# florasion/D-VQVAE

Measured on NVIDIA B200. Metric: vq_latents_per_sec, higher is better.
Workload: dtype f32

## Files before the change

### d-vqvae_b200/csrc/dvq_api.cu

```cuda
#include <dlfcn.h>
#include <stdarg.h>
#include <stdlib.h>
#include <string.h>

#include "dvq_common.cuh"

namespace dvq {

static thread_local char g_err[512] = "";

void set_error(const char* fmt, ...) {
  va_list ap;
  va_start(ap, fmt);
  vsnprintf(g_err, sizeof(g_err), fmt, ap);
  va_end(ap);
}

int fail(int code, const char* fmt, ...) {
  va_list ap;
  va_start(ap, fmt);
  vsnprintf(g_err, sizeof(g_err), fmt, ap);
  va_end(ap);
  return code;
}

int device_props(DeviceProps* out) {
  static DeviceProps cache[64];
  static bool have[64] = {};
  int dev = 0;
  DVQ_CUDA_CHECK(cudaGetDevice(&dev));
  if (dev < 0 || dev >= 64) return fail(DVQ_ERR_CUDA, "device ordinal %d out of range", dev);
  if (!have[dev]) {
    DeviceProps p;
    DVQ_CUDA_CHECK(cudaDeviceGetAttribute(&p.sm_count, cudaDevAttrMultiProcessorCount, dev));
    DVQ_CUDA_CHECK(cudaDeviceGetAttribute(&p.cc_major, cudaDevAttrComputeCapabilityMajor, dev));
    DVQ_CUDA_CHECK(cudaDeviceGetAttribute(&p.cc_minor, cudaDevAttrComputeCapabilityMinor, dev));
    DVQ_CUDA_CHECK(cudaDeviceGetAttribute(&p.max_smem_optin, cudaDevAttrMaxSharedMemoryPerBlockOptin, dev));
    cache[dev] = p;
    have[dev] = true;
  }
  *out = cache[dev];
  return DVQ_OK;
}

static long long g_launches = 0;
void count_launch(int n) { __atomic_fetch_add(&g_launches, (long long)n, __ATOMIC_RELAXED); }

static int g_refine_mode = 0;
static long long g_refine_pair_cap = 0;
long long refine_pair_cap_override() { return __atomic_load_n(&g_refine_pair_cap, __ATOMIC_RELAXED); }

static const int kStages = 4;
static const int kProfSlots = 128;
static thread_local bool g_prof_on = false;
static thread_local cudaEvent_t g_prof_ev[kStages][kProfSlots][2] = {};
static thread_local int g_prof_n[kStages] = {};

void profile_mark(int stage, bool begin, cudaStream_t s) {
  if (!g_prof_on || stage < 0 || stage >= kStages) return;
  const int slot = g_prof_n[stage];
  if (slot >= kProfSlots) return;
  cudaEvent_t& e = g_prof_ev[stage][slot][begin ? 0 : 1];
  if (!e && cudaEventCreate(&e) != cudaSuccess) return;
  cudaEventRecord(e, s);
  if (!begin) g_prof_n[stage] = slot + 1;
}

static int require_sm100() {
  DeviceProps dp;
  int rc = device_props(&dp);
  if (rc) return rc;
  if (dp.cc_major != 10)
    return fail(DVQ_ERR_UNSUPPORTED_ARCH, "libdvq_sm100 is built for sm_100a only; device is sm_%d%d",
                dp.cc_major, dp.cc_minor);
  return DVQ_OK;
}

VqWorkspace vq_workspace_layout(int64_t N, int K, int D, int flags) {
  VqWorkspace w;
  size_t off = 0;
  w.off_ee = off;
  off = align_up(off + sizeof(float) * (size_t)K, 256);
  w.off_counters = off;
  off = align_up(off + sizeof(int) * 64, 256);
  const bool may_tc = (flags & DVQ_PATH_MASK) != DVQ_PATH_SIMT && vq_tc_supported(N, K, D);
  w.off_rowlist = off;
  if (may_tc) off = align_up(off + 2 * align_up(sizeof(int) * (size_t)N, 256), 256);
  w.off_bop = off;
  if (may_tc) off = align_up(off + vq_tc_operand_bytes(K, D), 1024);
  w.off_binned = off;
  if (may_tc) off = align_up(off + vq_refine_binned_bytes(N), 256);
  w.total = off;
  return w;
}

}

using namespace dvq;

extern "C" {

int dvq_abi_version(void) { return DVQ_ABI_VERSION; }

const char* dvq_last_error(void) { return g_err; }

long long dvq_launch_count(void) { return __atomic_load_n(&g_launches, __ATOMIC_RELAXED); }

int dvq_vq_set_refine(int mode, long long pair_cap) {
  if (mode < 0 || mode > 2) return fail(DVQ_ERR_BAD_ARG, "refine mode must be 0 (auto), 1 (per-row) or 2 (binned)");
  __atomic_store_n(&g_refine_mode, mode, __ATOMIC_RELAXED);
  __atomic_store_n(&g_refine_pair_cap, pair_cap > 0 ? pair_cap : 0, __ATOMIC_RELAXED);
  return DVQ_OK;
}

int dvq_debug_tc_layout(int K, int D, int* out8) {
  if (!out8) return fail(DVQ_ERR_BAD_ARG, "out8 is NULL");
  if (K <= 0 || D <= 0) return fail(DVQ_ERR_BAD_SHAPE, "need K > 0, D > 0");
  vq_tc_layout_info(K, D, out8);
  return DVQ_OK;
}

int dvq_debug_tc_pair_layout(long long N, int K, int D, int* out8) {
  if (!out8) return fail(DVQ_ERR_BAD_ARG, "out8 is NULL");
  if (K <= 0 || D <= 0) return fail(DVQ_ERR_BAD_SHAPE, "need K > 0, D > 0");
  vq_tc_pair_layout_info((int64_t)N, K, D, out8);
  return DVQ_OK;
}

int dvq_debug_tc_layout_ex(long long N, int K, int D, int flags, int* out8) {
  if (!out8) return fail(DVQ_ERR_BAD_ARG, "out8 is NULL");
  if (K <= 0 || D <= 0) return fail(DVQ_ERR_BAD_SHAPE, "need K > 0, D > 0");
  const int zbytes = (flags & DVQ_Z_BF16) ? 2 : 4;
  if (vq_tc_pair_selected((int64_t)N, K, D)) vq_tc_pair_layout_info((int64_t)N, K, D, out8, zbytes);
  else vq_tc_layout_info(K, D, out8, zbytes);
  return DVQ_OK;
}

long long dvq_debug_tc_image_offset(int k, int d, int K, int D, int pair, long long* image_bytes) {
  if (K <= 0 || D <= 0 || k < 0 || k >= K || d < 0 || d >= D + 16 || !vq_tc_supported(1, K, D)) return -1;
  return vq_tc_image_offset(k, d, K, D, pair, image_bytes);
}

int dvq_profile_enable(int on) {
  g_prof_on = on != 0;
  for (int i = 0; i < kStages; ++i) g_prof_n[i] = 0;
  return DVQ_OK;
}

int dvq_profile_mean(float* ms, int* count, int n) {
  if (!ms || n <= 0) return fail(DVQ_ERR_BAD_ARG, "ms is NULL or n <= 0");
  for (int i = 0; i < n; ++i) {
    ms[i] = 0.f;
    if (count) count[i] = 0;
    if (i >= kStages) continue;
    double sum = 0.0;
    for (int j = 0; j < g_prof_n[i]; ++j) {
      float t = 0.f;
      DVQ_CUDA_CHECK(cudaEventSynchronize(g_prof_ev[i][j][1]));
      DVQ_CUDA_CHECK(cudaEventElapsedTime(&t, g_prof_ev[i][j][0], g_prof_ev[i][j][1]));
      sum += t;
    }
    if (g_prof_n[i] > 0) ms[i] = (float)(sum / g_prof_n[i]);
    if (count) count[i] = g_prof_n[i];
  }
  return DVQ_OK;
}

int dvq_device_info(int* sm_count, int* cc_major, int* cc_minor) {
  DeviceProps dp;
  int rc = device_props(&dp);
  if (rc) return rc;
  if (sm_count) *sm_count = dp.sm_count;
  if (cc_major) *cc_major = dp.cc_major;
  if (cc_minor) *cc_minor = dp.cc_minor;
  return DVQ_OK;
}

static int check_vq_shape(int64_t N, int K, int D) {
  if (N < 0 || K <= 0 || D <= 0) return fail(DVQ_ERR_BAD_SHAPE, "need N >= 0, K > 0, D > 0 (got N=%lld K=%d D=%d)", (long long)N, K, D);
  if (N > 2147483647LL - 256) return fail(DVQ_ERR_BAD_SHAPE, "N=%lld exceeds the per-call limit of 2^31-257 rows; shard the call", (long long)N);
  return DVQ_OK;
}

int dvq_vq_workspace_bytes(int64_t N, int K, int D, int flags, size_t* bytes) {
  if (!bytes) return fail(DVQ_ERR_BAD_ARG, "bytes is NULL");
  int rc = check_vq_shape(N, K, D);
  if (rc) return rc;
  *bytes = vq_workspace_layout(N, K, D, flags).total;
  return DVQ_OK;
}

int dvq_vq_forward(const float* z, const float* E, int64_t N, int K, int D, int flags, float* z_q, int64_t* idx,
                   float* onehot, unsigned long long* hist, double* sse, void* workspace, size_t workspace_bytes,
                   void* stream) {
  int rc = check_vq_shape(N, K, D);
  if (rc) return rc;
  const int train = (flags & DVQ_TRAIN) ? 1 : 0;
  if (!E || !workspace) return fail(DVQ_ERR_BAD_ARG, "E / workspace must not be NULL");
  if (N > 0 && (!z || !z_q || !idx)) return fail(DVQ_ERR_BAD_ARG, "z, z_q and idx must not be NULL");
  if (train && (!hist || !sse)) return fail(DVQ_ERR_BAD_ARG, "DVQ_TRAIN needs hist and sse");
  if ((flags & DVQ_WRITE_ONEHOT) && !onehot) return fail(DVQ_ERR_BAD_ARG, "DVQ_WRITE_ONEHOT needs onehot");
  const bool zbf = (flags & DVQ_Z_BF16) != 0;
  if ((reinterpret_cast<uintptr_t>(z) | reinterpret_cast<uintptr_t>(z_q)) % (zbf ? 2 : 4) != 0 || reinterpret_cast<uintptr_t>(E) % 4 != 0 ||
      reinterpret_cast<uintptr_t>(idx) % 8 != 0 || reinterpret_cast<uintptr_t>(workspace) % 256 != 0)
    return fail(DVQ_ERR_BAD_ALIGN, "z/z_q need %d-byte, E 4-byte, idx 8-byte, workspace 256-byte alignment", zbf ? 2 : 4);
  const VqWorkspace w = vq_workspace_layout(N, K, D, flags);
  if (workspace_bytes < w.total)
    return fail(DVQ_ERR_WORKSPACE, "workspace too small: %zu < %zu bytes", workspace_bytes, w.total);
  rc = require_sm100();
  if (rc) return rc;
  cudaStream_t s = static_cast<cudaStream_t>(stream);
  char* ws = static_cast<char*>(workspace);
  float* ee = reinterpret_cast<float*>(ws + w.off_ee);

  const int path = flags & DVQ_PATH_MASK;
  const bool tc_ok = vq_tc_supported(N, K, D);
  if (path == DVQ_PATH_TC && !tc_ok)
    return fail(DVQ_ERR_BAD_SHAPE, "DVQ_PATH_TC: shape N=%lld K=%d D=%d is not handled by the tcgen05 kernel", (long long)N, K, D);
  const bool aligned16 = (reinterpret_cast<uintptr_t>(z) | reinterpret_cast<uintptr_t>(E) | reinterpret_cast<uintptr_t>(z_q)) % 16 == 0;
  const bool use_tc = tc_ok && path != DVQ_PATH_SIMT && (aligned16 || path == DVQ_PATH_TC);

  const bool cached = (flags & DVQ_CODEBOOK_CACHED) != 0;
  profile_mark(0, true, s);
  if (!cached) rc = launch_code_norms(E, K, D, ee, s);
  profile_mark(0, false, s);
  if (rc) return rc;
  if (N > 0) {
    if (use_tc) {
      int* counters = reinterpret_cast<int*>(ws + w.off_counters);
      int* row_list = reinterpret_cast<int*>(ws + w.off_rowlist);
      int* cand_list = reinterpret_cast<int*>(ws + w.off_rowlist + align_up(sizeof(int) * (size_t)N, 256));
      profile_mark(1, true, s);
      rc = launch_vq_tc(z, E, ee, N, K, D, train, z_q, idx, hist, sse, ws + w.off_bop, counters, row_list, cand_list,
                        reinterpret_cast<int*>(ws + w.off_binned), (int)(vq_refine_binned_zero_bytes() / sizeof(int)), cached, zbf, s);
      profile_mark(1, false, s);
      if (rc) return rc;
      profile_mark(2, true, s);
      const bool list_mode = vq_tc_cand_gshift(K) < 0;
      if (vq_refine_supported(K, D)) {
        static const bool env_per_row = getenv("DVQ_REFINE_PER_ROW") != nullptr;
        static const bool env_binned = getenv("DVQ_REFINE_BINNED") != nullptr;
        const int mode = __atomic_load_n(&g_refine_mode, __ATOMIC_RELAXED);
        const bool force_per_row = env_per_row || mode == 1, force_binned = env_binned || mode == 2;
        const bool per_row_only = force_per_row || (!force_binned && vq_refine_codebook_in_smem(K, D));
        if (!per_row_only)
          rc = launch_vq_refine_binned(z, E, ee, N, K, D, train, z_q, idx, hist, sse, row_list, cand_list, counters, list_mode ? 1 : 0,
                                       ws + w.off_binned, zbf, s);
        if (!rc)
          rc = launch_vq_refine(z, E, ee, K, D, train, z_q, idx, hist, sse, row_list, cand_list, per_row_only ? counters : counters + 5,
                                vq_tc_cand_gshift(K), list_mode ? row_list + (N - 1) : nullptr,
                                list_mode ? (per_row_only ? counters + 2 : counters + 6) : nullptr, zbf, s);
      } else {
        rc = launch_vq_simt(z, E, ee, N, K, D, train, z_q, idx, hist, sse, row_list, counters, 1, zbf, s);
        if (!rc && list_mode)
          rc = launch_vq_simt(z, E, ee, N, K, D, train, z_q, idx, hist, sse, row_list + (N - 1), counters + 2, -1, zbf, s);
      }
      profile_mark(2, false, s);
      if (rc) return rc;
    } else {
      profile_mark(1, true, s);
      rc = launch_vq_simt(z, E, ee, N, K, D, train, z_q, idx, hist, sse, nullptr, nullptr, 1, zbf, s);
      profile_mark(1, false, s);
      if (rc) return rc;
    }
    if (flags & DVQ_WRITE_ONEHOT) {
      profile_mark(3, true, s);
      rc = launch_onehot(idx, N, K, onehot, s);
      profile_mark(3, false, s);
      if (rc) return rc;
    }
  }
  return DVQ_OK;
}

int dvq_vq_read_counters(const void* workspace, int64_t N, int K, int D, int flags, int* out4) {
  if (!workspace || !out4) return fail(DVQ_ERR_BAD_ARG, "NULL argument");
  int rc = check_vq_shape(N, K, D);
  if (rc) return rc;
  out4[0] = out4[1] = out4[2] = out4[3] = 0;
  const bool use_tc = vq_tc_supported(N, K, D) && (flags & DVQ_PATH_MASK) != DVQ_PATH_SIMT;
  if (!use_tc) return DVQ_OK;
  const VqWorkspace w = vq_workspace_layout(N, K, D, flags);
  DVQ_CUDA_CHECK(cudaMemcpy(out4, static_cast<const char*>(workspace) + w.off_counters, 4 * sizeof(int), cudaMemcpyDeviceToHost));
  if (getenv("DVQ_TC_STATS_PRINT")) {
    unsigned long long st[17];
    DVQ_CUDA_CHECK(cudaMemcpy(st, static_cast<const char*>(workspace) + w.off_counters + 32, sizeof(st), cudaMemcpyDeviceToHost));
    static const char* names[17] = {"producer.wait_stage_empty", "mma.wait_a_full", "mma.wait_acc_empty", "mma.total",
                                    "conv.wait_stage_full", "conv.wait_a_empty", "conv.total", "epi0.wait_acc_full",
                                    "epi4.wait_fin_empty", "epi0.wait_fin_full", "epi0.wait_sidx_empty", "epi0.total",
                                    "gather.wait_sidx_full", "gather.total", "mma.wait_b_full", "(unused)", "mma.wait_peer_acc_empty"};
    for (int i = 0; i < 17; ++i) fprintf(stderr, "[dvq tc stats] %-28s %14llu cycles (sum over CTAs)\n", names[i], st[i]);
    if (N >= 65536) {
      static long long tr[5 * 8 * 8];
      DVQ_CUDA_CHECK(cudaMemcpy(tr, static_cast<const char*>(workspace) + w.off_rowlist + (size_t)(N - 8192) * sizeof(int), sizeof(tr),
                                cudaMemcpyDeviceToHost));
      static const char* ev[5][4] = {{"mma.a_full", "mma.acc_empty", "mma.issued", "mma.complete"},
                                     {"own.acc_full", "own.chunk_done", "own.fin_full", "own.sidx_out"},
                                     {"hlp.acc_full", "hlp.chunk_done", "hlp.fin_out", "hlp.stage_freed"},
                                     {"cnv.stage_full", "cnv.pass1_done", "cnv.a_empty", "cnv.a_full_out"},
                                     {"gth.sidx_full", "gth.done", "", ""}};
      long long base = tr[(0 * 8 + 0) * 8 + 0];
      for (int role = 0; role < 5; ++role)
        for (int e = 0; e < 4; ++e) {
          if (!ev[role][e][0]) continue;
          fprintf(stderr, "[dvq tc trace] %-16s", ev[role][e]);
          for (int k = 0; k < 8; ++k) {
            const long long v = tr[(role * 8 + e) * 8 + k];
            fprintf(stderr, " %7lld", v ? v - base : -1);
          }
          fprintf(stderr, "\n");
        }
    }
  }
  return DVQ_OK;
}

int dvq_vq_finalize(const unsigned long long* hist, const double* sse, int64_t N_total, int K, int D, float al,
                    float beta, float* loss, float* perplexity, void* stream) {
  if (!hist || !sse || !loss || !perplexity) return fail(DVQ_ERR_BAD_ARG, "NULL argument");
  if (N_total < 0 || K <= 0 || D <= 0) return fail(DVQ_ERR_BAD_SHAPE, "need N_total >= 0 (0 = take the histogram total), K, D > 0");
  int rc = require_sm100();
  if (rc) return rc;
  return launch_finalize(hist, sse, N_total, K, D, al, beta, loss, perplexity, static_cast<cudaStream_t>(stream));
}

int dvq_gather(const float* E, const int64_t* idx, int64_t N, int K, int D, float* out, int* oob, void* stream) {
  if (N < 0 || K <= 0 || D <= 0) return fail(DVQ_ERR_BAD_SHAPE, "need N >= 0, K > 0, D > 0");
  if (N > 0 && (!E || !idx || !out)) return fail(DVQ_ERR_BAD_ARG, "NULL argument");
  int rc = require_sm100();
  if (rc) return rc;
  return launch_gather(E, idx, N, K, D, out, oob, static_cast<cudaStream_t>(stream));
}

int dvq_vq_backward_ex(const float* z, const float* E, const int64_t* idx, const float* g_zq, const float* g_loss,
                       const float* rows, int64_t N, int K, int D, float al, float beta, int flags, float* dz, float* dE,
                       void* stream) {
  if (N < 0 || K <= 0 || D <= 0 || (D & 3)) return fail(DVQ_ERR_BAD_SHAPE, "need N >= 0, K > 0, D a positive multiple of 4");
  if (flags & ~DVQ_Z_BF16) return fail(DVQ_ERR_BAD_ARG, "dvq_vq_backward_ex accepts DVQ_Z_BF16 only");
  if (!g_loss || !rows || (N > 0 && (!z || !E || !idx))) return fail(DVQ_ERR_BAD_ARG, "NULL argument");
  const bool zbf = (flags & DVQ_Z_BF16) != 0;
  if ((reinterpret_cast<uintptr_t>(E) | reinterpret_cast<uintptr_t>(dE)) % 16 != 0 ||
      (reinterpret_cast<uintptr_t>(z) | reinterpret_cast<uintptr_t>(g_zq) | reinterpret_cast<uintptr_t>(dz)) % (zbf ? 8 : 16) != 0)
    return fail(DVQ_ERR_BAD_ALIGN, "dvq_vq_backward needs 16-byte aligned E / dE and %d-byte aligned z / g_zq / dz", zbf ? 8 : 16);
  int rc = require_sm100();
  if (rc) return rc;
  return launch_vq_backward(z, E, idx, g_zq, g_loss, rows, N, D, al, beta, dz, dE, zbf, static_cast<cudaStream_t>(stream));
}

int dvq_vq_backward(const float* z, const float* E, const int64_t* idx, const float* g_zq, const float* g_loss,
                    const float* rows, int64_t N, int K, int D, float al, float beta, float* dz, float* dE, void* stream) {
  return dvq_vq_backward_ex(z, E, idx, g_zq, g_loss, rows, N, K, D, al, beta, 0, dz, dE, stream);
}

int dvq_vq_code_sums_ex(const float* z, const int64_t* idx, int64_t N, int K, int D, int flags, float* sums, void* stream) {
  if (N < 0 || K <= 0 || D <= 0 || (D & 3)) return fail(DVQ_ERR_BAD_SHAPE, "need N >= 0, K > 0, D a positive multiple of 4");
  if (flags & ~DVQ_Z_BF16) return fail(DVQ_ERR_BAD_ARG, "dvq_vq_code_sums_ex accepts DVQ_Z_BF16 only");
  if (N > 0 && (!z || !idx || !sums)) return fail(DVQ_ERR_BAD_ARG, "NULL argument");
  const bool zbf = (flags & DVQ_Z_BF16) != 0;
  if (reinterpret_cast<uintptr_t>(sums) % 16 != 0 || reinterpret_cast<uintptr_t>(z) % (zbf ? 8 : 16) != 0)
    return fail(DVQ_ERR_BAD_ALIGN, "dvq_vq_code_sums needs 16-byte aligned sums and a %d-byte aligned z", zbf ? 8 : 16);
  int rc = require_sm100();
  if (rc) return rc;
  return launch_vq_code_sums(z, idx, N, D, sums, zbf, static_cast<cudaStream_t>(stream));
}

int dvq_vq_code_sums(const float* z, const int64_t* idx, int64_t N, int K, int D, float* sums, void* stream) {
  return dvq_vq_code_sums_ex(z, idx, N, K, D, 0, sums, stream);
}

int dvq_gather_multi(const float* const* E, int G, const int64_t* codes, int64_t N, int K, int D, float* out, int64_t out_stride,
                     int* oob, void* stream) {
  if (G <= 0 || G > 8 || N < 0 || K <= 0 || D <= 0 || (D & 3) || out_stride < (int64_t)G * D || (out_stride & 3))
    return fail(DVQ_ERR_BAD_SHAPE, "need 1 <= G <= 8, D %% 4 == 0, out_stride >= G * D and a multiple of 4");
  if (!E || (N > 0 && (!codes || !out))) return fail(DVQ_ERR_BAD_ARG, "NULL argument");
  for (int g = 0; g < G; ++g)
    if (!E[g] || reinterpret_cast<uintptr_t>(E[g]) % 16) return fail(DVQ_ERR_BAD_ALIGN, "codebook %d is NULL or not 16-byte aligned", g);
  if (reinterpret_cast<uintptr_t>(out) % 16) return fail(DVQ_ERR_BAD_ALIGN, "out needs 16-byte alignment");
  int rc = require_sm100();
  if (rc) return rc;
  return launch_gather_multi(E, G, codes, N, K, D, out, out_stride, oob, static_cast<cudaStream_t>(stream));
}

int dvq_mano_forward(const DvqManoModel* model, const float* betas, const float* global_orient, const float* hand_pose,
                     const float* transl, int B, float* vertices, float* joints, void* stream) {
  if (B < 0) return fail(DVQ_ERR_BAD_SHAPE, "B must be >= 0");
  if (!model || (B > 0 && (!betas || !hand_pose || !vertices))) return fail(DVQ_ERR_BAD_ARG, "NULL argument");
  if (!model->v_template || !model->shapedirs || !model->posedirs || !model->j_regressor || !model->weights || !model->pose_mean ||
      !model->parents || (model->ncomps > 0 && !model->hands_components))
    return fail(DVQ_ERR_BAD_ARG, "DvqManoModel has a NULL table");
  if (model->ncomps < 0 || model->ncomps > 45) return fail(DVQ_ERR_BAD_SHAPE, "ncomps must be in [0, 45]");
  if (reinterpret_cast<uintptr_t>(model->weights) % 16) return fail(DVQ_ERR_BAD_ALIGN, "the skinning weights need 16-byte alignment");
  int rc = require_sm100();
  if (rc) return rc;
  return launch_mano(model, betas, global_orient, hand_pose, transl, B, vertices, joints, static_cast<cudaStream_t>(stream));
}

int dvq_pcnn_gemm(const DvqPcnnGemm* g, void* stream) {
  int rc = require_sm100();
  if (rc) return rc;
  return launch_pcnn_gemm(g, static_cast<cudaStream_t>(stream));
}

int dvq_pcnn_embed(const int64_t* x, int x_stride, int W, int B, int Bp, const float* emb, int n_emb, int d, void* img16,
                   float* img32, void* stream) {
  if (!x || !emb || !img16) return fail(DVQ_ERR_BAD_ARG, "NULL argument");
  if (W <= 0 || B <= 0 || Bp < B || Bp % 128 || d <= 0 || d % 8 || n_emb <= 0) return fail(DVQ_ERR_BAD_SHAPE, "need Bp %% 128 == 0, Bp >= B > 0, d %% 8 == 0");
  int rc = require_sm100();
  if (rc) return rc;
  return launch_pcnn_embed(x, x_stride, W, B, Bp, emb, n_emb, d, img16, img32, static_cast<cudaStream_t>(stream));
}

int dvq_pcnn_rows_to_image(const int64_t* label, int B, int Bp, const float* table, int n_rows, int kd, void* img16, void* stream) {
  if (!label || !table || !img16) return fail(DVQ_ERR_BAD_ARG, "NULL argument");
  if (B <= 0 || Bp < B || Bp % 128 || kd <= 0 || kd % 8 || n_rows <= 0) return fail(DVQ_ERR_BAD_SHAPE, "need Bp %% 128 == 0, Bp >= B > 0, kd %% 8 == 0");
  int rc = require_sm100();
  if (rc) return rc;
  return launch_pcnn_rows_to_image(label, B, Bp, table, n_rows, kd, img16, static_cast<cudaStream_t>(stream));
}

int dvq_debug_umma(const void* a_img, uint32_t a_bytes, const void* b_img, uint32_t b_bytes, int ksteps,
                   const uint32_t* strides, uint32_t idesc, int n_cols, float* out, int* err, void* stream) {
  if (!a_img || !b_img || !strides || !out || !err) return fail(DVQ_ERR_BAD_ARG, "NULL argument");
  if (a_bytes % 16 || b_bytes % 16 || n_cols % 32 || n_cols <= 0 || n_cols > 256 || ksteps <= 0)
    return fail(DVQ_ERR_BAD_SHAPE, "images must be multiples of 16 bytes, n_cols a multiple of 32 in (0,256]");
  if ((size_t)a_bytes + b_bytes > 200 * 1024) return fail(DVQ_ERR_BAD_SHAPE, "operand images exceed 200 KB");
  int rc = require_sm100();
  if (rc) return rc;
  return launch_umma_probe(a_img, a_bytes, b_img, b_bytes, ksteps, strides, idesc, n_cols, out, err, static_cast<cudaStream_t>(stream));
}

int dvq_onehot(const int64_t* idx, int64_t N, int K, float* out, void* stream) {
  if (N < 0 || K <= 0) return fail(DVQ_ERR_BAD_SHAPE, "need N >= 0, K > 0");
  if (N > 0 && (!idx || !out)) return fail(DVQ_ERR_BAD_ARG, "NULL argument");
  int rc = require_sm100();
  if (rc) return rc;
  return launch_onehot(idx, N, K, out, static_cast<cudaStream_t>(stream));
}

static int check_pn_shape(int B, int C, int P) {
  if (B < 0 || P <= 0 || (C != 3 && C != 4)) return fail(DVQ_ERR_BAD_SHAPE, "need B >= 0, P > 0, C in {3,4} (got B=%d C=%d P=%d)", B, C, P);
  return DVQ_OK;
}

int dvq_pointnet_workspace_bytes_ex(int B, int C, int P, int flags, size_t* bytes) {
  if (!bytes) return fail(DVQ_ERR_BAD_ARG, "bytes is NULL");
  int rc = check_pn_shape(B, C, P);
  if (rc) return rc;
  *bytes = pointnet_workspace_bytes(B, C, P, flags);
  return DVQ_OK;
}

int dvq_pointnet_workspace_bytes(int B, int C, int P, size_t* bytes) { return dvq_pointnet_workspace_bytes_ex(B, C, P, 0, bytes); }

int dvq_pointnet_forward_ex(const float* x, const DvqPointNetWeights* w, int B, int C, int P, int flags, float* feat,
                            float* trans, void* workspace, size_t workspace_bytes, void* stream) {
  int rc = check_pn_shape(B, C, P);
  if (rc) return rc;
  if (!w) return fail(DVQ_ERR_BAD_ARG, "weights struct is NULL");
  if (B > 0 && (!x || !feat || !trans || !workspace)) return fail(DVQ_ERR_BAD_ARG, "NULL argument");
  if (workspace_bytes < pointnet_workspace_bytes(B, C, P, flags))
    return fail(DVQ_ERR_WORKSPACE, "workspace too small: %zu < %zu bytes", workspace_bytes, pointnet_workspace_bytes(B, C, P, flags));
  rc = require_sm100();
  if (rc) return rc;
  if (B == 0) return DVQ_OK;
  return launch_pointnet(x, w, B, C, P, flags, feat, trans, workspace, workspace_bytes, static_cast<cudaStream_t>(stream));
}

int dvq_pointnet_forward(const float* x, const DvqPointNetWeights* w, int B, int C, int P, float* feat, float* trans,
                         void* workspace, size_t workspace_bytes, void* stream) {
  return dvq_pointnet_forward_ex(x, w, B, C, P, 0, feat, trans, workspace, workspace_bytes, stream);
}

struct DvqHostCtx {
  static const int kSlots = 3;
  int64_t chunk_rows;
  int K_max, D_max;
  cudaStream_t s_in, s_run, s_out;
  float* z_dev[kSlots];
  float* zq_dev[kSlots];
  int64_t* idx_dev[kSlots];
  cudaEvent_t ev_in[kSlots], ev_run[kSlots], ev_out[kSlots];
  float* E_dev;
  unsigned long long* hist_dev;
  double* sse_dev;
  float* scal_dev;
  void* ws;
  size_t ws_bytes;
};

int dvq_host_ctx_destroy(DvqHostCtx* c) {
  if (!c) return DVQ_OK;
  for (int i = 0; i < DvqHostCtx::kSlots; ++i) {
    if (c->z_dev[i]) cudaFree(c->z_dev[i]);
    if (c->zq_dev[i]) cudaFree(c->zq_dev[i]);
    if (c->idx_dev[i]) cudaFree(c->idx_dev[i]);
    if (c->ev_in[i]) cudaEventDestroy(c->ev_in[i]);
    if (c->ev_run[i]) cudaEventDestroy(c->ev_run[i]);
    if (c->ev_out[i]) cudaEventDestroy(c->ev_out[i]);
  }
  if (c->E_dev) cudaFree(c->E_dev);
  if (c->hist_dev) cudaFree(c->hist_dev);
  if (c->ws) cudaFree(c->ws);
  if (c->s_in) cudaStreamDestroy(c->s_in);
  if (c->s_run) cudaStreamDestroy(c->s_run);
  if (c->s_out) cudaStreamDestroy(c->s_out);
  free(c);
  return DVQ_OK;
}

int dvq_host_ctx_create(int64_t chunk_rows, int K_max, int D_max, DvqHostCtx** out) {
  if (!out) return fail(DVQ_ERR_BAD_ARG, "ctx out pointer is NULL");
  int rc = check_vq_shape(chunk_rows, K_max, D_max);
  if (rc) return rc;
  if (chunk_rows <= 0) return fail(DVQ_ERR_BAD_SHAPE, "chunk_rows must be positive");
  rc = require_sm100();
  if (rc) return rc;
  DvqHostCtx* c = static_cast<DvqHostCtx*>(calloc(1, sizeof(DvqHostCtx)));
  if (!c) return fail(DVQ_ERR_CUDA, "out of host memory");
  c->chunk_rows = chunk_rows;
  c->K_max = K_max;
  c->D_max = D_max;
#define CTX_CHECK(expr)                                                                     \
  do {                                                                                      \
    cudaError_t _e = (expr);                                                                \
    if (_e != cudaSuccess) {                                                                \
      dvq_host_ctx_destroy(c);                                                              \
      return fail(DVQ_ERR_CUDA, "%s failed: %s", #expr, cudaGetErrorString(_e));           \
    }                                                                                       \
  } while (0)
  CTX_CHECK(cudaStreamCreateWithFlags(&c->s_in, cudaStreamNonBlocking));
  CTX_CHECK(cudaStreamCreateWithFlags(&c->s_run, cudaStreamNonBlocking));
  CTX_CHECK(cudaStreamCreateWithFlags(&c->s_out, cudaStreamNonBlocking));
  const size_t row_bytes = sizeof(float) * (size_t)D_max;
  for (int i = 0; i < DvqHostCtx::kSlots; ++i) {
    CTX_CHECK(cudaMalloc(&c->z_dev[i], row_bytes * chunk_rows));
    CTX_CHECK(cudaMalloc(&c->zq_dev[i], row_bytes * chunk_rows));
    CTX_CHECK(cudaMalloc(&c->idx_dev[i], sizeof(int64_t) * chunk_rows));
    CTX_CHECK(cudaEventCreateWithFlags(&c->ev_in[i], cudaEventDisableTiming));
    CTX_CHECK(cudaEventCreateWithFlags(&c->ev_run[i], cudaEventDisableTiming));
    CTX_CHECK(cudaEventCreateWithFlags(&c->ev_out[i], cudaEventDisableTiming));
  }
  CTX_CHECK(cudaMalloc(&c->E_dev, row_bytes * K_max));
  const size_t stat_bytes = align_up(sizeof(unsigned long long) * (size_t)K_max, 16) + 32;
  CTX_CHECK(cudaMalloc(&c->hist_dev, stat_bytes));
  c->sse_dev = reinterpret_cast<double*>(reinterpret_cast<char*>(c->hist_dev) + align_up(sizeof(unsigned long long) * (size_t)K_max, 16));
  c->scal_dev = reinterpret_cast<float*>(c->sse_dev + 1);
  size_t ws_need = 0;
  for (int k = 32; ; k *= 2) {
    const int kk = k < K_max ? k : K_max;
    for (int d = 16; ; d *= 2) {
      const int dd = d < D_max ? d : D_max;
      const size_t t = vq_workspace_layout(chunk_rows, kk, dd, 0).total;
      ws_need = t > ws_need ? t : ws_need;
      if (dd == D_max) break;
    }
    if (kk == K_max) break;
  }
  c->ws_bytes = ws_need + 4096;
  CTX_CHECK(cudaMalloc(&c->ws, c->ws_bytes));
#undef CTX_CHECK
  *out = c;
  return DVQ_OK;
}

int dvq_vq_forward_host(DvqHostCtx* c, const float* z_host, const float* E_host, int64_t N, int K, int D, int flags,
                        float al, float beta, float* zq_host, int64_t* idx_host, float* loss_host,
                        float* perplexity_host) {
  if (!c) return fail(DVQ_ERR_BAD_ARG, "ctx is NULL");
  int rc = check_vq_shape(N, K, D);
  if (rc) return rc;
  if (K > c->K_max || D > c->D_max)
    return fail(DVQ_ERR_BAD_SHAPE, "K=%d D=%d exceed the context limits K_max=%d D_max=%d", K, D, c->K_max, c->D_max);
  if (flags & DVQ_WRITE_ONEHOT) return fail(DVQ_ERR_BAD_ARG, "the host-buffer entry does not materialise the one-hot matrix");
  if (flags & DVQ_Z_BF16) return fail(DVQ_ERR_BAD_ARG, "the host-buffer entry takes fp32 rows only (DVQ_Z_BF16 is not accepted)");
  if (!E_host || (N > 0 && (!z_host || !zq_host || !idx_host))) return fail(DVQ_ERR_BAD_ARG, "NULL host pointer");
  const int train = (flags & DVQ_TRAIN) ? 1 : 0;
  if (train && (!loss_host || !perplexity_host)) return fail(DVQ_ERR_BAD_ARG, "DVQ_TRAIN needs loss_host and perplexity_host");
  const int64_t chunk = c->chunk_rows;
  const size_t row_bytes = sizeof(float) * (size_t)D;

  DVQ_CUDA_CHECK(cudaMemcpyAsync(c->E_dev, E_host, row_bytes * K, cudaMemcpyHostToDevice, c->s_in));
  cudaEvent_t ev_E = c->ev_in[0];
  DVQ_CUDA_CHECK(cudaEventRecord(ev_E, c->s_in));
  DVQ_CUDA_CHECK(cudaStreamWaitEvent(c->s_run, ev_E, 0));
  if (train)
    DVQ_CUDA_CHECK(cudaMemsetAsync(c->hist_dev, 0, align_up(sizeof(unsigned long long) * (size_t)c->K_max, 16) + 32, c->s_run));

  int64_t n_chunks = (N + chunk - 1) / chunk;
  for (int64_t ci = 0; ci < n_chunks; ++ci) {
    const int b = (int)(ci % DvqHostCtx::kSlots);
    const int64_t r0 = ci * chunk;
    const int64_t rows = (N - r0 < chunk) ? (N - r0) : chunk;
    if (ci >= DvqHostCtx::kSlots) {
      DVQ_CUDA_CHECK(cudaStreamWaitEvent(c->s_in, c->ev_run[b], 0));
      DVQ_CUDA_CHECK(cudaStreamWaitEvent(c->s_run, c->ev_out[b], 0));
    }
    DVQ_CUDA_CHECK(cudaMemcpyAsync(c->z_dev[b], z_host + r0 * D, row_bytes * rows, cudaMemcpyHostToDevice, c->s_in));
    DVQ_CUDA_CHECK(cudaEventRecord(c->ev_in[b], c->s_in));
    DVQ_CUDA_CHECK(cudaStreamWaitEvent(c->s_run, c->ev_in[b], 0));
    if (!(flags & DVQ_HOST_COPY_ONLY)) {
      const int cflags = flags | ((ci > 0 && rows == chunk) ? DVQ_CODEBOOK_CACHED : 0);
      rc = dvq_vq_forward(c->z_dev[b], c->E_dev, rows, K, D, cflags, c->zq_dev[b], c->idx_dev[b], nullptr, c->hist_dev,
                          c->sse_dev, c->ws, c->ws_bytes, c->s_run);
      if (rc) return rc;
    }
    DVQ_CUDA_CHECK(cudaEventRecord(c->ev_run[b], c->s_run));
    DVQ_CUDA_CHECK(cudaStreamWaitEvent(c->s_out, c->ev_run[b], 0));
    DVQ_CUDA_CHECK(cudaMemcpyAsync(zq_host + r0 * D, c->zq_dev[b], row_bytes * rows, cudaMemcpyDeviceToHost, c->s_out));
    DVQ_CUDA_CHECK(cudaMemcpyAsync(idx_host + r0, c->idx_dev[b], sizeof(int64_t) * rows, cudaMemcpyDeviceToHost, c->s_out));
    DVQ_CUDA_CHECK(cudaEventRecord(c->ev_out[b], c->s_out));
  }
  float scal[2] = {0.f, 0.f};
  if (train && N > 0 && !(flags & DVQ_HOST_COPY_ONLY)) {
    rc = launch_finalize(c->hist_dev, c->sse_dev, N, K, D, al, beta, c->scal_dev, c->scal_dev + 1, c->s_run);
    if (rc) return rc;
    DVQ_CUDA_CHECK(cudaMemcpyAsync(scal, c->scal_dev, sizeof(scal), cudaMemcpyDeviceToHost, c->s_run));
  }
  DVQ_CUDA_CHECK(cudaStreamSynchronize(c->s_in));
  DVQ_CUDA_CHECK(cudaStreamSynchronize(c->s_run));
  DVQ_CUDA_CHECK(cudaStreamSynchronize(c->s_out));
  if (train) {
    *loss_host = scal[0];
    *perplexity_host = scal[1];
  }
  return DVQ_OK;
}

typedef int (*nccl_allreduce_fn)(const void*, void*, size_t, int, int, void*, cudaStream_t);
typedef int (*nccl_group_fn)(void);
typedef const char* (*nccl_errstr_fn)(int);

int dvq_allreduce_stats(void* nccl_comm, unsigned long long* hist, double* sse, int K, void* stream) {
  static nccl_allreduce_fn p_allreduce = nullptr;
  static nccl_group_fn p_start = nullptr, p_end = nullptr;
  static nccl_errstr_fn p_err = nullptr;
  if (!nccl_comm || !hist || !sse || K <= 0) return fail(DVQ_ERR_BAD_ARG, "NULL communicator / buffer or K <= 0");
  if (!p_allreduce) {
    const char* override_path = getenv("DVQ_NCCL_LIB");
    void* h = nullptr;
    if (override_path) h = dlopen(override_path, RTLD_NOW | RTLD_GLOBAL);
    if (!h) h = dlopen("libnccl.so.2", RTLD_NOW | RTLD_NOLOAD);
    if (!h) h = dlopen("libnccl.so.2", RTLD_NOW | RTLD_GLOBAL);
    if (!h) h = dlopen("libnccl.so", RTLD_NOW | RTLD_GLOBAL);
    if (!h) return fail(DVQ_ERR_NCCL, "libnccl not found (set DVQ_NCCL_LIB): %s", dlerror());
    p_allreduce = reinterpret_cast<nccl_allreduce_fn>(dlsym(h, "ncclAllReduce"));
    p_start = reinterpret_cast<nccl_group_fn>(dlsym(h, "ncclGroupStart"));
    p_end = reinterpret_cast<nccl_group_fn>(dlsym(h, "ncclGroupEnd"));
    p_err = reinterpret_cast<nccl_errstr_fn>(dlsym(h, "ncclGetErrorString"));
    if (!p_allreduce || !p_start || !p_end) {
      p_allreduce = nullptr;
      return fail(DVQ_ERR_NCCL, "libnccl is missing ncclAllReduce/ncclGroupStart/ncclGroupEnd");
    }
  }
  const int kUint64 = 5, kFloat64 = 8, kSum = 0;
  cudaStream_t s = static_cast<cudaStream_t>(stream);
  int r = p_start();
  if (!r) r = p_allreduce(hist, hist, (size_t)K, kUint64, kSum, nccl_comm, s);
  if (!r) r = p_allreduce(sse, sse, 1, kFloat64, kSum, nccl_comm, s);
  int r2 = p_end();
  if (!r) r = r2;
  if (r) return fail(DVQ_ERR_NCCL, "NCCL all-reduce failed: %s", p_err ? p_err(r) : "unknown");
  return DVQ_OK;
}

}
```

### d-vqvae_b200/csrc/dvq_common.cuh

```cuda
#pragma once

#include <cuda_bf16.h>
#include <cuda_runtime.h>
#include <stdint.h>
#include <stdio.h>

#include "dvq.h"

namespace dvq {

void set_error(const char* fmt, ...);
int fail(int code, const char* fmt, ...);

#define DVQ_CUDA_CHECK(expr)                                                              \
  do {                                                                                    \
    cudaError_t _e = (expr);                                                              \
    if (_e != cudaSuccess)                                                                \
      return ::dvq::fail(DVQ_ERR_CUDA, "%s failed: %s (%s:%d)", #expr, cudaGetErrorString(_e), \
                         __FILE__, __LINE__);                                             \
  } while (0)

struct DeviceProps {
  int sm_count;
  int cc_major;
  int cc_minor;
  int max_smem_optin;
};
int device_props(DeviceProps* out);

void count_launch(int n = 1);
void profile_mark(int stage, bool begin, cudaStream_t s);

static inline size_t align_up(size_t x, size_t a) { return (x + a - 1) / a * a; }

struct VqWorkspace {
  size_t off_ee;
  size_t off_counters;
  size_t off_rowlist;
  size_t off_bop;
  size_t off_binned;
  size_t total;
};
VqWorkspace vq_workspace_layout(int64_t N, int K, int D, int flags);

int launch_code_norms(const float* E, int K, int D, float* ee, cudaStream_t s);

int launch_vq_simt(const void* z, const float* E, const float* ee, int64_t N, int K, int D, int train,
                   void* z_q, int64_t* idx, unsigned long long* hist, double* sse,
                   const int* row_list, const int* n_list, int list_stride, bool zbf, cudaStream_t s);

bool vq_tc_supported(int64_t N, int K, int D);
void vq_tc_layout_info(int K, int D, int* out8, int zbytes = 4);
bool vq_tc_pair_selected(int64_t N, int K, int D);
void vq_tc_pair_layout_info(int64_t N, int K, int D, int* out8, int zbytes = 4);
long long vq_tc_image_offset(int k, int d, int K, int D, int pair, long long* image_bytes);
size_t vq_tc_operand_bytes(int K, int D);
int launch_vq_tc(const void* z, const float* E, const float* ee, int64_t N, int K, int D, int train,
                 void* z_q, int64_t* idx, unsigned long long* hist, double* sse,
                 void* bop, int* counters, int* row_list, int* cand_list, int* zero_ints, int zero_n,
                 bool codebook_cached, bool zbf, cudaStream_t s);

bool vq_refine_supported(int K, int D);
bool vq_refine_codebook_in_smem(int K, int D);
int vq_tc_cand_gshift(int K);
int launch_vq_refine(const void* z, const float* E, const float* ee, int K, int D, int train, void* z_q, int64_t* idx,
                     unsigned long long* hist, double* sse, const int* row_list, const int* cand_list,
                     const int* n_list, int gshift, const int* ovf_last, const int* n_ovf, bool zbf, cudaStream_t s);

long long refine_pair_cap_override();
size_t vq_refine_binned_bytes(int64_t N);
size_t vq_refine_binned_zero_bytes();
int launch_vq_refine_binned(const void* z, const float* E, const float* ee, int64_t N, int K, int D, int train, void* z_q,
                            int64_t* idx, unsigned long long* hist, double* sse, const int* row_list, const int* cand_list,
                            int* counters, int list_mode, void* ws, bool zbf, cudaStream_t s);

int launch_onehot(const int64_t* idx, int64_t N, int K, float* onehot, cudaStream_t s);
int launch_finalize(const unsigned long long* hist, const double* sse, int64_t N, int K, int D, float al,
                    float beta, float* loss, float* ppl, cudaStream_t s);
int launch_vq_backward(const void* z, const float* E, const int64_t* idx, const void* g_zq, const float* g_loss,
                       const float* rows, int64_t N, int D, float al, float beta, void* dz, float* dE, bool zbf, cudaStream_t s);
int launch_gather_multi(const float* const* E, int G, const int64_t* codes, int64_t N, int K, int D, float* out, int64_t out_stride,
                        int* oob, cudaStream_t s);
int launch_vq_code_sums(const void* z, const int64_t* idx, int64_t N, int D, float* sums, bool zbf, cudaStream_t s);
int launch_gather(const float* E, const int64_t* idx, int64_t N, int K, int D, float* out, int* oob,
                  cudaStream_t s);

int launch_umma_probe(const void* a_img, uint32_t a_bytes, const void* b_img, uint32_t b_bytes, int ksteps,
                      const uint32_t* strides, uint32_t idesc, int n_cols, float* out, int* err, cudaStream_t s);

int launch_pcnn_gemm(const DvqPcnnGemm* g, cudaStream_t s);
int launch_pcnn_embed(const int64_t* x, int x_stride, int W, int B, int Bp, const float* emb, int n_emb, int d, void* img16,
                      float* img32, cudaStream_t s);
int launch_pcnn_rows_to_image(const int64_t* label, int B, int Bp, const float* table, int n_rows, int kd, void* img16, cudaStream_t s);

int launch_mano(const DvqManoModel* m, const float* betas, const float* global_orient, const float* hand_pose, const float* transl, int B,
                float* vertices, float* joints, cudaStream_t s);

size_t pointnet_workspace_bytes(int B, int C, int P, int flags);
int launch_pointnet(const float* x, const DvqPointNetWeights* w, int B, int C, int P, int flags, float* feat,
                    float* trans, void* ws, size_t ws_bytes, cudaStream_t s);
size_t pointnet_tc_image_bytes();
int launch_pointnet_tc_trunk(const float* x, const float* trans, const float* w1, const float* b1, const float* w2,
                             const float* b2, const float* w3, int B, int C, int P, float* maxbuf, void* images,
                             bool main_trunk, cudaStream_t s);

__device__ __forceinline__ float4 ldg4(const float* p) { return __ldg(reinterpret_cast<const float4*>(p)); }

__device__ __forceinline__ float zf(float v) { return v; }
__device__ __forceinline__ float zf(__nv_bfloat16 v) { return __bfloat162float(v); }
__device__ __forceinline__ float4 bf4_to_f4(uint2 u) {
  return make_float4(__uint_as_float(u.x << 16), __uint_as_float(u.x & 0xffff0000u), __uint_as_float(u.y << 16),
                     __uint_as_float(u.y & 0xffff0000u));
}
__device__ __forceinline__ uint32_t f2_to_bf2(float lo, float hi) {
  const __nv_bfloat162 h = __floats2bfloat162_rn(lo, hi);
  return *reinterpret_cast<const uint32_t*>(&h);
}
__device__ __forceinline__ uint2 f4_to_bf4(float4 v) { return make_uint2(f2_to_bf2(v.x, v.y), f2_to_bf2(v.z, v.w)); }
__device__ __forceinline__ float4 zld4(const float* p) { return *reinterpret_cast<const float4*>(p); }
__device__ __forceinline__ float4 zld4(const __nv_bfloat16* p) { return bf4_to_f4(*reinterpret_cast<const uint2*>(p)); }
__device__ __forceinline__ float4 zldg4(const float* p) { return __ldg(reinterpret_cast<const float4*>(p)); }
__device__ __forceinline__ float4 zldg4(const __nv_bfloat16* p) { return bf4_to_f4(__ldg(reinterpret_cast<const uint2*>(p))); }
__device__ __forceinline__ float4 zldcs4(const float* p) { return __ldcs(reinterpret_cast<const float4*>(p)); }
__device__ __forceinline__ float4 zldcs4(const __nv_bfloat16* p) { return bf4_to_f4(__ldcs(reinterpret_cast<const uint2*>(p))); }
__device__ __forceinline__ void zst4(float* p, float4 v) { *reinterpret_cast<float4*>(p) = v; }
__device__ __forceinline__ void zst4(__nv_bfloat16* p, float4 v) { *reinterpret_cast<uint2*>(p) = f4_to_bf4(v); }
__device__ __forceinline__ void zstcs4(float* p, float4 v) { __stcs(reinterpret_cast<float4*>(p), v); }
__device__ __forceinline__ void zstcs4(__nv_bfloat16* p, float4 v) { __stcs(reinterpret_cast<uint2*>(p), f4_to_bf4(v)); }
__device__ __forceinline__ void zst1(float* p, float v) { *p = v; }
__device__ __forceinline__ void zst1(__nv_bfloat16* p, float v) { *p = __float2bfloat16_rn(v); }

__device__ __forceinline__ double warp_sum(double v) {
#pragma unroll
  for (int o = 16; o > 0; o >>= 1) v += __shfl_xor_sync(0xffffffffu, v, o);
  return v;
}
__device__ __forceinline__ float warp_sum(float v) {
#pragma unroll
  for (int o = 16; o > 0; o >>= 1) v += __shfl_xor_sync(0xffffffffu, v, o);
  return v;
}

}
```

Baseline: 5.940 billion.

## Add code-stationary refine kernel holding codebook in registers across rows

Adds a new refine kernel in which each thread keeps one codebook vector in registers while tiles of candidate rows are streamed into shared memory with cp.async double buffering. Each warp evaluates its 32 codes against the rows whose candidate mask selects it, then a block-level min reduction produces the final index, z_q, histogram and SSE. It becomes the default for mask-mode K of at least 128 (at least 256 when D is 128) that fits the warp limit, replacing the per-row and binned refine paths. This trades register pressure and single-block occupancy for reuse of codebook data across many rows.

```diff
diff --git a/d-vqvae_b200/csrc/dvq_api.cu b/d-vqvae_b200/csrc/dvq_api.cu
--- a/d-vqvae_b200/csrc/dvq_api.cu
+++ b/d-vqvae_b200/csrc/dvq_api.cu
@@ -107,7 +107,7 @@
 long long dvq_launch_count(void) { return __atomic_load_n(&g_launches, __ATOMIC_RELAXED); }
 
 int dvq_vq_set_refine(int mode, long long pair_cap) {
-  if (mode < 0 || mode > 2) return fail(DVQ_ERR_BAD_ARG, "refine mode must be 0 (auto), 1 (per-row) or 2 (binned)");
+  if (mode < 0 || mode > 3) return fail(DVQ_ERR_BAD_ARG, "refine mode must be 0 (auto), 1 (per-row), 2 (binned) or 3 (code-stationary)");
   __atomic_store_n(&g_refine_mode, mode, __ATOMIC_RELAXED);
   __atomic_store_n(&g_refine_pair_cap, pair_cap > 0 ? pair_cap : 0, __ATOMIC_RELAXED);
   return DVQ_OK;
@@ -242,11 +242,14 @@
         static const bool env_binned = getenv("DVQ_REFINE_BINNED") != nullptr;
         const int mode = __atomic_load_n(&g_refine_mode, __ATOMIC_RELAXED);
         const bool force_per_row = env_per_row || mode == 1, force_binned = env_binned || mode == 2;
+        const bool stationary = mode == 3 || (!force_per_row && !force_binned && vq_refine_stationary_default(K, D));
         const bool per_row_only = force_per_row || (!force_binned && vq_refine_codebook_in_smem(K, D));
-        if (!per_row_only)
+        if (stationary)
+          rc = launch_vq_refine_stationary(z, E, ee, K, D, train, z_q, idx, hist, sse, row_list, cand_list, counters, zbf, s);
+        else if (!per_row_only)
           rc = launch_vq_refine_binned(z, E, ee, N, K, D, train, z_q, idx, hist, sse, row_list, cand_list, counters, list_mode ? 1 : 0,
                                        ws + w.off_binned, zbf, s);
-        if (!rc)
+        if (!rc && !stationary)
           rc = launch_vq_refine(z, E, ee, K, D, train, z_q, idx, hist, sse, row_list, cand_list, per_row_only ? counters : counters + 5,
                                 vq_tc_cand_gshift(K), list_mode ? row_list + (N - 1) : nullptr,
                                 list_mode ? (per_row_only ? counters + 2 : counters + 6) : nullptr, zbf, s);
diff --git a/d-vqvae_b200/csrc/dvq_common.cuh b/d-vqvae_b200/csrc/dvq_common.cuh
--- a/d-vqvae_b200/csrc/dvq_common.cuh
+++ b/d-vqvae_b200/csrc/dvq_common.cuh
@@ -66,6 +66,12 @@
 int launch_vq_refine(const void* z, const float* E, const float* ee, int K, int D, int train, void* z_q, int64_t* idx,
                      unsigned long long* hist, double* sse, const int* row_list, const int* cand_list,
                      const int* n_list, int gshift, const int* ovf_last, const int* n_ovf, bool zbf, cudaStream_t s);
+
+bool vq_refine_stationary_supported(int K, int D);
+bool vq_refine_stationary_default(int K, int D);
+int launch_vq_refine_stationary(const void* z, const float* E, const float* ee, int K, int D, int train, void* z_q, int64_t* idx,
+                                unsigned long long* hist, double* sse, const int* row_list, const int* cand_list,
+                                const int* n_list, bool zbf, cudaStream_t s);
 
 long long refine_pair_cap_override();
 size_t vq_refine_binned_bytes(int64_t N);
diff --git a/d-vqvae_b200/csrc/vq_refine_stationary.cu b/d-vqvae_b200/csrc/vq_refine_stationary.cu
--- /dev/null
+++ b/d-vqvae_b200/csrc/vq_refine_stationary.cu
@@ -0,0 +1,262 @@
+#include "dvq_common.cuh"
+
+namespace dvq {
+namespace {
+
+constexpr int SB = 128;
+constexpr int SMAX_WARPS = 31;
+constexpr uint32_t KEY_INF = 0xff800000u;
+
+template <int DT>
+constexpr int stationary_max_warps() { return DT <= 16 ? 31 : DT <= 64 ? 16 : DT == 128 ? 8 : 0; }
+
+__device__ __forceinline__ uint32_t dist_key(float d) {
+  if (!(d == d)) d = INFINITY;
+  const uint32_t b = __float_as_uint(d);
+  return (b & 0x80000000u) ? ~b : (b | 0x80000000u);
+}
+
+template <int R, int DT, typename ZT>
+__device__ __forceinline__ void eval_rows(const float (&e)[DT], float eek, int sc_base, const ZT* __restrict__ zb,
+                                          const unsigned char* rs, const float* s_zz, unsigned long long* cand, int lane) {
+  int r[R];
+  float acc[R];
+#pragma unroll
+  for (int i = 0; i < R; ++i) { r[i] = rs[i]; acc[i] = 0.f; }
+#pragma unroll
+  for (int d = 0; d < DT; d += 4) {
+#pragma unroll
+    for (int i = 0; i < R; ++i) {
+      const float4 z4 = zld4(zb + r[i] * DT + d);
+      acc[i] = fmaf(z4.x, e[d], acc[i]);
+      acc[i] = fmaf(z4.y, e[d + 1], acc[i]);
+      acc[i] = fmaf(z4.z, e[d + 2], acc[i]);
+      acc[i] = fmaf(z4.w, e[d + 3], acc[i]);
+    }
+  }
+#pragma unroll
+  for (int i = 0; i < R; ++i) {
+    const uint32_t key = dist_key(__fmaf_rn(-2.0f, acc[i], __fadd_rn(s_zz[r[i]], eek)));
+    const uint32_t kmin = __reduce_min_sync(0xffffffffu, key);
+    const int src = __ffs(__ballot_sync(0xffffffffu, key == kmin)) - 1;
+    if (lane == 0) cand[r[i]] = ((unsigned long long)kmin << 32) | (unsigned)(sc_base + src);
+  }
+}
+
+template <int DT, typename ZT>
+__global__ void __launch_bounds__(stationary_max_warps<DT>() * 32, 1)
+vq_refine_stationary_kernel(const ZT* __restrict__ z, const float* __restrict__ E, const float* __restrict__ ee, int K, int train,
+                            ZT* __restrict__ zq, int64_t* __restrict__ idx_out, unsigned long long* __restrict__ hist,
+                            double* __restrict__ sse, const int* __restrict__ row_list, const int* __restrict__ cand_list,
+                            const int* __restrict__ n_list) {
+  extern __shared__ __align__(16) unsigned char smem_raw[];
+  ZT* zbuf = reinterpret_cast<ZT*>(smem_raw);
+  unsigned long long* s_cand = reinterpret_cast<unsigned long long*>(smem_raw + 2 * SB * DT * sizeof(ZT));
+  __shared__ int s_row[3][SB];
+  __shared__ unsigned s_mask[3][SB];
+  __shared__ float s_zz[SB];
+  __shared__ int s_bidx[SB];
+  __shared__ unsigned char s_list[SMAX_WARPS][SB];
+  __shared__ unsigned s_hist[SMAX_WARPS * 32];
+  __shared__ double s_sse[SMAX_WARPS];
+  constexpr int ZE = 16 / (int)sizeof(ZT);
+  constexpr int PPR = DT / ZE;
+  constexpr int C4 = DT / 4;
+  const int nt = blockDim.x, nw = nt >> 5;
+  const int tid = threadIdx.x, warp = tid >> 5, lane = tid & 31;
+  uint32_t lanemask_lt;
+  asm("mov.u32 %0, %%lanemask_lt;" : "=r"(lanemask_lt));
+  const int n = *n_list;
+  const int start = (int)((int64_t)n * blockIdx.x / gridDim.x);
+  const int end = (int)((int64_t)n * (blockIdx.x + 1) / gridDim.x);
+  if (start >= end) return;
+  const int nb = (end - start + SB - 1) / SB;
+
+  auto stage_ids = [&](int b) {
+    const int i0 = start + b * SB, cnt = min(SB, end - i0);
+    for (int t = tid; t < cnt; t += nt) {
+      const uint32_t dr = (uint32_t)__cvta_generic_to_shared(&s_row[b % 3][t]);
+      const uint32_t dm = (uint32_t)__cvta_generic_to_shared(&s_mask[b % 3][t]);
+      asm volatile("cp.async.ca.shared.global [%0], [%1], 4;" ::"r"(dr), "l"(row_list + i0 + t) : "memory");
+      asm volatile("cp.async.ca.shared.global [%0], [%1], 4;" ::"r"(dm), "l"(cand_list + i0 + t) : "memory");
+    }
+  };
+  auto stage_z = [&](int b) {
+    const int cnt = min(SB, end - (start + b * SB));
+    const int* rows = s_row[b % 3];
+    ZT* dst0 = zbuf + (b & 1) * SB * DT;
+    for (int p = tid; p < cnt * PPR; p += nt) {
+      const int r = p / PPR, c = p - r * PPR;
+      const uint32_t dst = (uint32_t)__cvta_generic_to_shared(dst0 + r * DT + c * ZE);
+      asm volatile("cp.async.cg.shared.global [%0], [%1], 16;" ::"r"(dst), "l"(z + (int64_t)rows[r] * DT + c * ZE) : "memory");
+    }
+  };
+
+  stage_ids(0);
+  asm volatile("cp.async.commit_group;" ::: "memory");
+  const int code = warp * 32 + lane;
+  float e[DT];
+#pragma unroll
+  for (int d = 0; d < DT; d += 4) {
+    const float4 v = ldg4(E + (int64_t)code * DT + d);
+    e[d] = v.x; e[d + 1] = v.y; e[d + 2] = v.z; e[d + 3] = v.w;
+  }
+  const float eek = __ldg(ee + code);
+  if (train) {
+    for (int k = tid; k < K; k += nt) s_hist[k] = 0u;
+    if (lane == 0) s_sse[warp] = 0.0;
+  }
+  asm volatile("cp.async.wait_group 0;" ::: "memory");
+  __syncthreads();
+  stage_z(0);
+  if (nb > 1) stage_ids(1);
+  asm volatile("cp.async.commit_group;" ::: "memory");
+
+  for (int b = 0; b < nb; ++b) {
+    const int cnt = min(SB, end - (start + b * SB));
+    asm volatile("cp.async.wait_group 0;" ::: "memory");
+    __syncthreads();
+    if (b + 1 < nb) {
+      stage_z(b + 1);
+      if (b + 2 < nb) stage_ids(b + 2);
+    }
+    asm volatile("cp.async.commit_group;" ::: "memory");
+    const ZT* zb = zbuf + (b & 1) * SB * DT;
+    const int* rows = s_row[b % 3];
+    const unsigned* masks = s_mask[b % 3];
+    for (int r0 = warp; r0 < cnt; r0 += 4 * nw) {
+      float s2[4];
+#pragma unroll
+      for (int u = 0; u < 4; ++u) {
+        const int r = min(r0 + u * nw, cnt - 1);
+        s2[u] = 0.f;
+#pragma unroll
+        for (int c = 0; c < DT; c += 32) {
+          if (c + lane < DT) { const float v = zf(zb[r * DT + c + lane]); s2[u] = fmaf(v, v, s2[u]); }
+        }
+      }
+#pragma unroll
+      for (int u = 0; u < 4; ++u) s2[u] = warp_sum(s2[u]);
+      if (lane == 0) {
+#pragma unroll
+        for (int u = 0; u < 4; ++u)
+          if (r0 + u * nw < cnt) s_zz[r0 + u * nw] = s2[u];
+      }
+    }
+    for (int i = tid; i < nw * SB; i += nt) s_cand[i] = ~0ull;
+    __syncthreads();
+    unsigned char* list = s_list[warp];
+    int m = 0;
+    for (int g = 0; g < cnt; g += 32) {
+      const int r = g + lane;
+      const unsigned mk = r < cnt ? masks[r] : 1u;
+      const bool sel = r < cnt && (mk == 0u || ((mk >> warp) & 1u));
+      const unsigned bal = __ballot_sync(0xffffffffu, sel);
+      if (sel) list[m + __popc(bal & lanemask_lt)] = (unsigned char)r;
+      m += __popc(bal);
+    }
+    __syncwarp();
+    unsigned long long* cand = s_cand + warp * SB;
+    int j = 0;
+    for (; j + 4 <= m; j += 4) eval_rows<4, DT>(e, eek, warp * 32, zb, list + j, s_zz, cand, lane);
+    if (j + 2 <= m) { eval_rows<2, DT>(e, eek, warp * 32, zb, list + j, s_zz, cand, lane); j += 2; }
+    if (j < m) eval_rows<1, DT>(e, eek, warp * 32, zb, list + j, s_zz, cand, lane);
+    __syncthreads();
+    for (int r = tid; r < cnt; r += nt) {
+      unsigned long long best = ~0ull;
+      for (int w = 0; w < nw; ++w) best = min(best, s_cand[w * SB + r]);
+      const int bidx = (uint32_t)(best >> 32) >= KEY_INF ? 0 : (int)(uint32_t)best;
+      s_bidx[r] = bidx;
+      idx_out[rows[r]] = (int64_t)bidx;
+      if (train) atomicAdd(s_hist + bidx, 1u);
+    }
+    __syncthreads();
+    double lsse = 0.0;
+#pragma unroll 4
+    for (int p = tid; p < cnt * C4; p += nt) {
+      const int r = p / C4, c = (p - r * C4) * 4;
+      const float4 e4 = ldg4(E + (int64_t)s_bidx[r] * DT + c);
+      float4 o4 = e4;
+      if (train) {
+        const float4 z4 = zld4(zb + r * DT + c);
+        const float dx = __fsub_rn(e4.x, z4.x), dy = __fsub_rn(e4.y, z4.y);
+        const float dz = __fsub_rn(e4.z, z4.z), dw = __fsub_rn(e4.w, z4.w);
+        lsse += (double)dx * dx + (double)dy * dy + (double)dz * dz + (double)dw * dw;
+        o4 = make_float4(__fadd_rn(z4.x, dx), __fadd_rn(z4.y, dy), __fadd_rn(z4.z, dz), __fadd_rn(z4.w, dw));
+      }
+      zst4(zq + (int64_t)rows[r] * DT + c, o4);
+    }
+    if (train) {
+      lsse = warp_sum(lsse);
+      if (lane == 0) s_sse[warp] += lsse;
+    }
+  }
+  if (train) {
+    __syncthreads();
+    for (int k = tid; k < K; k += nt)
+      if (s_hist[k]) atomicAdd(hist + k, (unsigned long long)s_hist[k]);
+    if (lane == 0 && s_sse[warp] != 0.0) atomicAdd(sse, s_sse[warp]);
+  }
+}
+
+template <int DT, typename ZT>
+int launch_stationary_dt(const ZT* z, const float* E, const float* ee, int K, int train, ZT* z_q, int64_t* idx,
+                         unsigned long long* hist, double* sse, const int* row_list, const int* cand_list, const int* n_list,
+                         int sm_count, cudaStream_t s) {
+  auto kern = vq_refine_stationary_kernel<DT, ZT>;
+  const int threads = K;
+  const size_t bytes = (size_t)2 * SB * DT * sizeof(ZT) + (size_t)(K / 32) * SB * sizeof(unsigned long long);
+  DVQ_CUDA_CHECK(cudaFuncSetAttribute(kern, cudaFuncAttributeMaxDynamicSharedMemorySize, (int)bytes));
+  int per_sm = 0;
+  DVQ_CUDA_CHECK(cudaOccupancyMaxActiveBlocksPerMultiprocessor(&per_sm, kern, threads, bytes));
+  kern<<<sm_count * (per_sm > 0 ? per_sm : 1), threads, bytes, s>>>(z, E, ee, K, train, z_q, idx, hist, sse, row_list, cand_list, n_list);
+  DVQ_CUDA_CHECK(cudaGetLastError());
+  count_launch();
+  return DVQ_OK;
+}
+
+template <typename ZT>
+int launch_stationary_t(const ZT* z, const float* E, const float* ee, int K, int D, int train, ZT* z_q, int64_t* idx,
+                        unsigned long long* hist, double* sse, const int* row_list, const int* cand_list, const int* n_list,
+                        int sm_count, cudaStream_t s) {
+  switch (D) {
+    case 16: return launch_stationary_dt<16>(z, E, ee, K, train, z_q, idx, hist, sse, row_list, cand_list, n_list, sm_count, s);
+    case 32: return launch_stationary_dt<32>(z, E, ee, K, train, z_q, idx, hist, sse, row_list, cand_list, n_list, sm_count, s);
+    case 64: return launch_stationary_dt<64>(z, E, ee, K, train, z_q, idx, hist, sse, row_list, cand_list, n_list, sm_count, s);
+    case 128: return launch_stationary_dt<128>(z, E, ee, K, train, z_q, idx, hist, sse, row_list, cand_list, n_list, sm_count, s);
+    default: return fail(DVQ_ERR_BAD_SHAPE, "code-stationary refine kernel is instantiated for e_dim 16..128 only");
+  }
+}
+
+}
+
+bool vq_refine_stationary_supported(int K, int D) {
+  int max_warps = 0;
+  switch (D) {
+    case 16: max_warps = stationary_max_warps<16>(); break;
+    case 32: max_warps = stationary_max_warps<32>(); break;
+    case 64: max_warps = stationary_max_warps<64>(); break;
+    case 128: max_warps = stationary_max_warps<128>(); break;
+    default: return false;
+  }
+  return vq_tc_cand_gshift(K) == 0 && K % 32 == 0 && K >= 32 && K / 32 <= max_warps;
+}
+
+bool vq_refine_stationary_default(int K, int D) { return vq_refine_stationary_supported(K, D) && K >= (D <= 64 ? 128 : 256); }
+
+int launch_vq_refine_stationary(const void* z, const float* E, const float* ee, int K, int D, int train, void* z_q, int64_t* idx,
+                                unsigned long long* hist, double* sse, const int* row_list, const int* cand_list,
+                                const int* n_list, bool zbf, cudaStream_t s) {
+  if (!vq_refine_stationary_supported(K, D))
+    return fail(DVQ_ERR_BAD_SHAPE, "code-stationary refine: K=%d, e_dim %d does not fit (mask-mode K with K/32 warps x e_dim registers)", K, D);
+  DeviceProps dp;
+  int rc = device_props(&dp);
+  if (rc) return rc;
+  if (zbf)
+    return launch_stationary_t(static_cast<const __nv_bfloat16*>(z), E, ee, K, D, train, static_cast<__nv_bfloat16*>(z_q), idx, hist,
+                               sse, row_list, cand_list, n_list, dp.sm_count, s);
+  return launch_stationary_t(static_cast<const float*>(z), E, ee, K, D, train, static_cast<float*>(z_q), idx, hist, sse, row_list,
+                             cand_list, n_list, dp.sm_count, s);
+}
+
+}
```

Result: faster. 6.143 billion, median of 6 (+3.4%).
